# YuvalNirkin/hyperseg

Measured on AMD Instinct MI355X. Metric: frames/sec @ bs=1 HyperSeg-M 1024x512, higher is better.
Workload: dtype f32 storage and accumulation; level-4 inverted residual products as 3-term f16 splits (f32-class: 1.3e-7 of sum|a||b|; exact_f32 beside it)

## Files before the change

hyperseg_amd/_hip.py:

```python
import ctypes as C
import os

import torch

_LIB_PATH = os.environ.get('HS_HIP_LIB') or os.path.join(os.path.dirname(os.path.abspath(__file__)), 'lib',
                                                         'libhyperseg_hip.so')

ACT_NONE, ACT_RELU, ACT_RELU6, ACT_SWISH = 0, 1, 2, 3
PAD_MODES = {'zeros': 0, 'reflect': 1, 'replicate': 2, 'circular': 3}
PREV_NONE, PREV_SAME, PREV_BILINEAR = 0, 1, 2

_STATUS = {-1: 'bad argument', -2: 'feature map does not tile into the weight grid (H % fh or W % fw != 0)',
           -3: 'unsupported shape', -4: 'tile does not fit the LDS'}


class HipLibraryError(RuntimeError):
    pass


class StageInputC(C.Structure):
    _fields_ = [('skip', C.c_void_p), ('prev', C.c_void_p),
                ('batch', C.c_int32), ('H', C.c_int32), ('W', C.c_int32),
                ('c_skip', C.c_int32), ('c_prev', C.c_int32),
                ('Hp', C.c_int32), ('Wp', C.c_int32),
# ... 150 lines not shown
        'hs_frame_rotate_fwd': ([vp, i32, i32, i32, i32, vp, i32, i32, C.c_uint32, C.c_uint32, vp, vp, vp], C.c_int),
        'hs_label_rotate_fwd': ([vp, i32, i32, i32, i32, vp, i32, i32, i32, i32, vp, i32, vp], C.c_int),
        'hs_resize_tables_ragged_fwd': ([vp, i32, i32, i32, i32, i32, i32, i32, vp, vp, vp, vp, vp], C.c_int),
        'hs_color_jitter_ragged_fwd': ([vp, i32, i32, i32, i32, vp, vp, vp, vp, vp], C.c_int),
        'hs_frame_resize_ragged_fwd': ([vp, i32, i32, i32, i32, vp, vp, vp, vp, i32, i32, i32, vp, vp], C.c_int),
        'hs_label_resize_ragged_fwd': ([vp, i32, i32, i32, i32, vp, vp, vp, i32, i32, vp, vp], C.c_int),
        'hs_frame_rotate_ragged_fwd': ([vp, i32, i32, i32, i32, vp, vp, vp, i32, i32, C.c_uint32, C.c_uint32, vp, vp, vp], C.c_int),
        'hs_label_rotate_ragged_fwd': ([vp, i32, i32, i32, vp, vp, vp, i32, i32, i32, i32, vp, i32, vp], C.c_int),
        'hs_mbconv_expand_dw_fwd': ([vp, i32, i32, i32, i32, vp, i32, vp, vp, vp, i32, i32, i32, i32, i32, i32, vp, vp, vp, vp, vp], C.c_int),
        'hs_se_gate_fwd': ([vp, i32, i32, i32, C.c_float, vp, vp, i32, vp, vp, vp, vp, vp, i32, vp, vp, vp], C.c_int),
        'hs_gemm_split_kp': ([i32], C.c_int),
        'hs_gemm_split_fwd': ([vp, vp, vp, vp, vp, i32, vp, vp, i32, i32, i32, i32, i32, vp], C.c_int),
        'hs_gemm_split_conv2x2_fwd': ([vp, vp, vp, vp, i32, vp, vp, i32, i32, i32, i32, i32, i32, vp], C.c_int),
        'hs_gemm_split_up2_fwd': ([vp, vp, vp, vp, i32, vp, i32, i32, i32, i32, i32, i32, vp], C.c_int),
        'hs_pooled_shift_fwd': ([vp, i32, C.c_float, vp, vp, vp, i32, i32, vp], C.c_int),
    }
    for name, (argtypes, restype) in sig.items():
        fn = getattr(lib, name)
        fn.argtypes, fn.restype = argtypes, restype
    if lib.hs_version() != 1:
        raise HipLibraryError(f'ABI mismatch: library reports version {lib.hs_version()}, binding expects 1')
    return lib


lib = _load()
EXPORTS = ['hs_version', 'hs_build_info', 'hs_signal2weights_fwd', 'hs_signal2weights_multi_fwd', 'hs_s2w_pack_floats', 'hs_s2w_pack_fwd', 'hs_bank_pack_fwd', 'hs_bn_fold_fwd',
           'hs_patch_conv_fwd', 'hs_patch_conv_s2w_fwd', 'hs_k1_chain_workspace', 'hs_k1_chain_fwd', 'hs_decoder_chain_workspace', 'hs_decoder_chain_fwd', 'hs_meta_conv_fwd', 'hs_meta_conv_bwd', 'hs_patch_conv_gen_fwd', 'hs_patch_ir_fwd', 'hs_patch_ir_v0_fwd', 'hs_patch_ir_v0_ws_fwd', 'hs_patch_ir_v0_workspace', 'hs_patch_ir_route', 'hs_ir_tile_map', 'hs_upsample_bilinear_fwd', 'hs_upsample_argmax_fwd',
           'hs_stage_input_fwd', 'hs_depthwise_conv_fwd', 'hs_depthwise_pool_blocks', 'hs_stem_conv_fwd', 'hs_stem_dw_fwd', 'hs_mbconv_tiles', 'hs_mbconv_expand_dw_fwd', 'hs_se_gate_fwd', 'hs_depthwise_conv_se_fwd', 'hs_mbconv_expand_dw_se_fwd', 'hs_se_tail_workspace', 'hs_se_tail_tails', 'hs_mbconv_se_workgroups', 'hs_pointwise_conv_fwd', 'hs_affine_act_fwd', 'hs_gemm_split_kp', 'hs_gemm_split_fwd', 'hs_gemm_split_conv2x2_fwd', 'hs_gemm_split_up2_fwd', 'hs_pooled_shift_fwd', 'hs_patch_conv_bwd_input',
           'hs_patch_conv_bwd_weight', 'hs_halo_tiles_fwd', 'hs_halo_tiles_bwd', 'hs_tile_interior_fwd', 'hs_tile_interior_bwd', 'hs_dw_tiles_fwd', 'hs_dw_tiles_bwd_in', 'hs_dw_tiles_bwd_w',
           'hs_s2w_train_fwd', 'hs_s2w_train_workspace', 'hs_s2w_train_bwd', 'hs_cross_entropy_fwd', 'hs_cross_entropy_bwd', 'hs_cross_entropy_typed_fwd', 'hs_cross_entropy_typed_bwd', 'hs_bootstrapped_ce_fwd', 'hs_bootstrapped_ce_bwd', 'hs_bootstrap_mean_workspace', 'hs_bootstrap_mean_fwd', 'hs_bootstrap_mean_bwd', 'hs_bootstrap_mean_batched_fwd', 'hs_bootstrap_mean_batched_bwd', 'hs_bn_train_workspace', 'hs_bn_train_stats_fwd', 'hs_dw_tiles_bn_fwd', 'hs_dw_tiles_bn_bwd_w', 'hs_patch_conv_bn_fwd', 'hs_patch_conv_bn_bwd_w', 'hs_adam_blocks', 'hs_adam_step', 'hs_bootstrap_mean_of_batch_fwd', 'hs_bootstrap_mean_of_batch_bwd', 'hs_upsample_bilinear_bwd', 'hs_upsample_bilinear_typed_bwd', 'hs_upsample_bilinear_bf16_fwd', 'hs_stage_input_typed_fwd', 'hs_bank_unpack_fwd', 'hs_bn_act_train_fwd',
           'hs_bn_act_train_bwd', 'hs_dw_tiles_bn_bwd_in_partials', 'hs_dw_tiles_bn_bwd_in', 'hs_bn_act_train_bwd_apply', 'hs_patch_conv_plain_fwd', 'hs_patch_conv_plain_bwd_in', 'hs_patch_conv_plain_bwd_w',
           'hs_upsample_bilinear_f16_fwd', 'hs_adam_step_amp', 'hs_eval_max_classes', 'hs_upsample_confusion_fwd', 'hs_confusion_fwd', 'hs_upsample2_confusion_fwd',
           'hs_image_ingest_fwd', 'hs_stem_dw_u8_fwd', 'hs_overlay_fwd', 'hs_upsample_overlay_fwd',
           'hs_frame_resize_fwd', 'hs_label_resize_fwd', 'hs_resize_tables_fwd', 'hs_frame_resize_batch_fwd', 'hs_label_resize_batch_fwd', 'hs_color_jitter_fwd', 'hs_frame_rotate_fwd', 'hs_label_rotate_fwd',
           'hs_resize_tables_ragged_fwd', 'hs_color_jitter_ragged_fwd', 'hs_frame_resize_ragged_fwd', 'hs_label_resize_ragged_fwd', 'hs_frame_rotate_ragged_fwd', 'hs_label_rotate_ragged_fwd',
           'hs_cross_entropy_score_fwd', 'hs_upsample_ce_confusion_fwd']


def check(status, what):
    if status == 0:
        return
    if status < 0:
        raise HipLibraryError(f'{what}: {_STATUS.get(status, status)}')
    raise HipLibraryError(f'{what}: HIP launch failed with hipError_t {status}')


def dev_ptr(t, name='tensor', dtype=torch.float32):
    if t is None:
        return None
    if not isinstance(t, torch.Tensor):
        raise TypeError(f'{name} must be a torch.Tensor')
# ... 30 lines not shown
```

hyperseg_amd/csrc/hs_gemm_split.hip:

```cpp
#include "hs_common.h"
#include <type_traits>

namespace hs {

using half8 = __attribute__((ext_vector_type(8))) _Float16;
using gs_f32x4 = __attribute__((ext_vector_type(4))) float;

__device__ __forceinline__ int gs_exp_of(float m) { return min(max(__float_as_int(m) >> 23, 27), 254); }
__device__ __forceinline__ float gs_scale_of(int eb) { return __int_as_float((268 - eb) << 23); }
__device__ __forceinline__ float gs_inv_scale_of(int eb) { return __int_as_float((eb - 14) << 23); }

struct GemmSplitArgs {
    const _Float16* __restrict__ wf;
    const float* __restrict__ w_inv;
    const float* __restrict__ gate; const float* __restrict__ x;
    const float* shift;
    const float* residual;
    float* y;
    int M, K, KST, N, act;
    int conv_wo;
    float* pool_partial;
    int up2_wo;
};

#ifndef HS_GS_NARROW_MAX_WG
#define HS_GS_NARROW_MAX_WG 128
#endif

#ifndef HS_GS_TALL_MIN_WG
#define HS_GS_TALL_MIN_WG 257
#endif

template <int KS, int NWV, bool FAST, int NS, int MT, int NCH, bool PATCH>
__global__ __launch_bounds__(64 * NWV)
void gemm_split_kernel(GemmSplitArgs a) {
    extern __shared__ __attribute__((aligned(16))) float gs_red[];
    constexpr int nthr = 64 * NWV, nwv = NWV;
    constexpr int NP = 16 * NS, NR = 16 * MT, NE = NR * NP;
    const int tid = threadIdx.x, lane = tid & 63, wave = tid >> 6;
    const int lrow = lane & 15, kg = lane >> 4;
    const int n0 = blockIdx.x * NP, r0 = blockIdx.y * MT, b = blockIdx.z;
    const float* __restrict__ xb = a.x + (size_t)b * a.K * a.N;
    const float* __restrict__ gb = a.gate ? a.gate + (size_t)b * a.K : nullptr;
    float* yb = a.y + (size_t)b * a.M * a.N * (a.up2_wo > 0 ? 4 : 1);
    const float* rb = a.residual ? a.residual + (size_t)b * a.M * a.N : nullptr;
    const int rt_max = (a.M + 15) >> 4;

    using gs_f32x2 = __attribute__((ext_vector_type(2))) float;
    const int ncol0 = min(n0 + NS * lrow, a.N - (FAST && !PATCH && NS == 2 ? 2 : 1)), ncol1 = min(n0 + NS * lrow + 1, a.N - 1);
    float xv[NCH][NS][KS][8];
    if constexpr (PATCH) {
        const int oy = ncol0 / a.conv_wo, ox = ncol0 - oy * a.conv_wo;
        const float* __restrict__ win = xb + (size_t)(2 * oy) * (2 * a.conv_wo) + 2 * ox;
        const int cmax = (a.K >> 2) - 1;
#pragma unroll
        for (int c = 0; c < NCH; ++c)
#pragma unroll
            for (int s = 0; s < KS; ++s)
#pragma unroll
// ... 149 lines not shown
                }
            }
            if (q + 2 < NCH * MT) { load_a(q + 2); __builtin_amdgcn_sched_barrier(0); }
#pragma unroll
            for (int t = 0; t < NS; ++t) {
#pragma unroll
                for (int r = 0; r < 4; ++r) {
                    const float v = c == 0 ? acc[t][r] * invb[t] : fmaf(acc[t][r], invb[t], tot[mt][t][r]);
                    if (c == NCH - 1) gs_red[(wave * NR + 16 * mt + 4 * kg + r) * NP + NS * lrow + t] = v;
                    else tot[mt][t][r] = v;
                }
            }
        }
    }
    __syncthreads();
    auto tail = [&](auto act_kind) {
        constexpr int ACT = decltype(act_kind)::value;
#pragma unroll
        for (int i = 0; i < TE; ++i) {
            const int e = tid + i * nthr;
            if (e < NE) {
                const int row = 16 * r0 + e / NP, col = n0 + (e & (NP - 1));
                float t = 0.0f;
#pragma unroll
                for (int w = 0; w < nwv; ++w) t += gs_red[w * NE + e];
                const bool live = row < a.M && col < a.N;
                float v = fmaf(t, wi[i], sh[i]);
                if constexpr (ACT == HS_ACT_SWISH) v = swishf(v);
                else if constexpr (ACT == HS_ACT_RELU) v = fmaxf(v, 0.0f);
                else if constexpr (ACT == HS_ACT_RELU6) v = fminf(fmaxf(v, 0.0f), 6.0f);
                v += yo[i];
                if (live) {
                    if (a.up2_wo > 0) {
                        const int oy = col / a.up2_wo, ox = col - oy * a.up2_wo;
                        float* dst = yb + (size_t)row * (4 * a.N) + (size_t)(2 * oy) * (2 * a.up2_wo) + 2 * ox;
                        *reinterpret_cast<gs_f32x2*>(dst) = gs_f32x2{v, v};
                        *reinterpret_cast<gs_f32x2*>(dst + 2 * a.up2_wo) = gs_f32x2{v, v};
                    } else {
                        yb[(size_t)row * a.N + col] = v;
                    }
                }
                if constexpr (NP == 16) {
                    if (a.pool_partial) {
                        const float rs = rowsum16(live ? v : 0.0f);
                        if ((e & 15) == 0 && row < a.M) a.pool_partial[((size_t)b * a.M + row) * gridDim.x + blockIdx.x] = rs;
                    }
                }
            }
        }
    };
    if (a.act == HS_ACT_SWISH) tail(std::integral_constant<int, HS_ACT_SWISH>{});
    else if (a.act == HS_ACT_NONE) tail(std::integral_constant<int, HS_ACT_NONE>{});
    else if (a.act == HS_ACT_RELU) tail(std::integral_constant<int, HS_ACT_RELU>{});
    else tail(std::integral_constant<int, HS_ACT_RELU6>{});
}

__global__ __launch_bounds__(256)
void pooled_shift_kernel(const float* __restrict__ partial, int nblk, float inv_p, const float* __restrict__ wb,
                         const float* __restrict__ shift, float* __restrict__ out, int M, int C) {
    extern __shared__ float ps_mean[];
    const int tid = threadIdx.x, lane = tid & 63, wave = tid >> 6;
    for (int c = tid; c < C; c += 256) {
        float t = 0.0f;
        for (int j = 0; j < nblk; ++j) t += partial[(size_t)c * nblk + j];
        ps_mean[c] = t * inv_p;
    }
    __syncthreads();
    const int r0 = 16 * blockIdx.x + 4 * wave;
    float acc[4] = {0.f, 0.f, 0.f, 0.f};
// ... 20 lines not shown
    return ks <= 5;
}

}

using namespace hs;

extern "C" int hs_gemm_split_kp(int32_t c_in) {
    int nwv, ks, nch;
    if (c_in <= 0 || !gemm_split_plan(c_in, nwv, ks, nch)) return HS_ERR_UNSUPPORTED;
    return nwv * nch * ks * 32;
}

static int launch_gemm_split_plain(const void* w_frag, const float* w_inv, const float* gate, const float* x, const float* shift,
                                   int32_t act, const float* residual, float* y, int32_t batch, int32_t c_out, int32_t c_in,
                                   int32_t kp, int32_t pixels, int up2_wo, void* stream) {
    if (!w_frag || !w_inv || !x || !y || batch <= 0 || c_out <= 0 || c_in <= 0 || pixels <= 0) return HS_ERR_BAD_ARG;
    if (act < 0 || act > 3) return HS_ERR_BAD_ARG;
    int nwv, ks, nch;
    if (!gemm_split_plan(c_in, nwv, ks, nch)) return HS_ERR_UNSUPPORTED;
    if (kp != nwv * nch * ks * 32 || (ks > 1 && nwv != 8)) return HS_ERR_BAD_ARG;
    if (batch > 65535 || (c_out + 31) / 32 > 65535) return HS_ERR_UNSUPPORTED;
    GemmSplitArgs a{(const _Float16*)w_frag, w_inv, gate, x, shift, residual, y, c_out, c_in, kp / 32, pixels, act, 0, nullptr, up2_wo};
    dim3 grid((pixels + 31) / 32, ((c_out + 15) / 16 + 1) / 2, batch);
    const size_t wgs = (size_t)grid.x * grid.y * grid.z;
    const bool narrow = wgs <= HS_GS_NARROW_MAX_WG && pixels > 16;
    const bool tall = wgs >= HS_GS_TALL_MIN_WG && c_out > 32;
    if (narrow) grid.x = (pixels + 15) / 16;
    if (tall) grid.y = ((c_out + 15) / 16 + 3) / 4;
    const size_t lds = (size_t)nwv * (narrow ? 512 : tall ? 2048 : 1024) * sizeof(float);
    hipStream_t s = (hipStream_t)stream;
    const bool fast = (c_in & 7) == 0 && (pixels & 1) == 0 && c_in >= 8;
#define HS_GS_(KSV, NWV, F) do { \
        if (narrow) hipLaunchKernelGGL((gemm_split_kernel<KSV, NWV, F, 1, 2, 1, false>), grid, dim3(64 * NWV), lds, s, a); \
        else if (tall) hipLaunchKernelGGL((gemm_split_kernel<KSV, NWV, F, 2, 4, 1, false>), grid, dim3(64 * NWV), lds, s, a); \
        else hipLaunchKernelGGL((gemm_split_kernel<KSV, NWV, F, 2, 2, 1, false>), grid, dim3(64 * NWV), lds, s, a); } while (0)
#define HS_GS(KSV, NWV) do { if (fast) HS_GS_(KSV, NWV, true); else HS_GS_(KSV, NWV, false); } while (0)
    if (nch == 2) {
        if (!fast || up2_wo > 0) return HS_ERR_UNSUPPORTED;
        grid.x = (pixels + 15) / 16; grid.y = ((c_out + 15) / 16 + 1) / 2;
        const size_t lds2 = (size_t)8 * 512 * sizeof(float);
#define HS_GS2(KSV) hipLaunchKernelGGL((gemm_split_kernel<KSV, 8, true, 1, 2, 2, false>), grid, dim3(512), lds2, s, a)
        switch (ks) { case 3: HS_GS2(3); break; case 4: HS_GS2(4); break; case 5: HS_GS2(5); break; default: return HS_ERR_UNSUPPORTED; }
#undef HS_GS2
        return launch_status();
    }
    switch (ks) {
        case 1: if (nwv == 2) HS_GS(1, 2); else if (nwv == 4) HS_GS(1, 4); else HS_GS(1, 8); break;
        case 2: HS_GS(2, 8); break;
        case 3: HS_GS(3, 8); break;
        case 4: HS_GS(4, 8); break;
        default: HS_GS(5, 8); break;
// ... 2 lines not shown
#undef HS_GS_
    return launch_status();
}

extern "C" int hs_gemm_split_fwd(const void* w_frag, const float* w_inv, const float* gate, const float* x,
                                 const float* shift, int32_t act, const float* residual, float* y,
                                 int32_t batch, int32_t c_out, int32_t c_in, int32_t kp, int32_t pixels, void* stream) {
    return launch_gemm_split_plain(w_frag, w_inv, gate, x, shift, act, residual, y, batch, c_out, c_in, kp, pixels, 0, stream);
}

extern "C" int hs_gemm_split_up2_fwd(const void* w_frag, const float* w_inv, const float* x, const float* shift, int32_t act,
                                     float* y, int32_t batch, int32_t c_out, int32_t c_in, int32_t kp, int32_t Ho, int32_t Wo,
                                     void* stream) {
    if (Ho <= 0 || Wo <= 0 || (((size_t)y) & 7) != 0) return HS_ERR_BAD_ARG;
    return launch_gemm_split_plain(w_frag, w_inv, nullptr, x, shift, act, nullptr, y, batch, c_out, c_in, kp, Ho * Wo, Wo, stream);
}

extern "C" int hs_pooled_shift_fwd(const float* partial, int32_t nblk, float inv_pixels, const float* wb, const float* shift,
                                   float* shift_out, int32_t rows, int32_t channels, void* stream) {
    if (!partial || !wb || !shift || !shift_out || nblk <= 0 || rows <= 0 || channels <= 0) return HS_ERR_BAD_ARG;
    if (channels > 8192) return HS_ERR_UNSUPPORTED;
    hipLaunchKernelGGL(pooled_shift_kernel, dim3((rows + 15) / 16), dim3(256), (size_t)channels * sizeof(float), (hipStream_t)stream,
                       partial, nblk, inv_pixels, wb, shift, shift_out, rows, channels);
    return launch_status();
}

extern "C" int hs_gemm_split_conv2x2_fwd(const void* w_frag, const float* w_inv, const float* x, const float* shift, int32_t act,
                                         float* y, float* pool_partial, int32_t batch, int32_t c_out, int32_t c_in, int32_t kp,
                                         int32_t Ho, int32_t Wo, void* stream) {
    if (!w_frag || !w_inv || !x || !y || batch <= 0 || c_out <= 0 || c_in <= 0 || Ho <= 0 || Wo <= 0) return HS_ERR_BAD_ARG;
// ... 27 lines not shown
```

hyperseg_amd/functional.py:

```python
import collections
import ctypes as C
import functools
import os
import threading

import torch

from . import _hip
from ._hip import ACT_NONE, ACT_RELU, ACT_RELU6, PAD_MODES

BN_EPS_DEFAULT = 1e-5
DTYPE_CODES = {torch.float32: 0, torch.bfloat16: 1, torch.float16: 2}
S2W_TRAIN_MAX_LAYERS = 8
COSCHEDULE_BANKS = os.environ.get('HS_COSCHEDULE_BANKS', '0') == '1'


def _round_up(n, m):
    return (n + m - 1) // m * m


def _device_of(a):
    if isinstance(a, torch.Tensor):
        return a.device
    if isinstance(a, (StageInput, BankRef, SignalRef, U8Frame)):
# ... 1036 lines not shown
        raise ValueError(f'input has {cin} channels, the weight {sw.c_in}')
    shape = (b, sw.c_out, 2 * h, 2 * w)
    if out is None:
        out = torch.empty(shape, device=x.device, dtype=torch.float32)
    elif tuple(out.shape) != shape:
        raise ValueError(f'out has shape {tuple(out.shape)}, expected {shape}')
    if shift is not None and shift.numel() != sw.c_out:
        raise ValueError(f'shift has {shift.numel()} entries, expected {sw.c_out}')
    st = _hip.lib.hs_gemm_split_up2_fwd(_hip.dev_ptr(sw.frag, 'w_frag', torch.float16), _hip.dev_ptr(sw.inv, 'w_inv'),
                                        _hip.dev_ptr(x, 'x'), _hip.dev_ptr(shift, 'shift') if shift is not None else None,
                                        int(act), _hip.dev_ptr(out, 'out'), b, sw.c_out, cin, sw.kp, h, w, _hip.stream_ptr())
    _hip.check(st, 'hs_gemm_split_up2_fwd')
    return out


@_on_operand_device
def pooled_shift(pool_partial, pixels, wb, shift):
    _, c, nblk = pool_partial.shape
    m = shift.numel()
    if pool_partial.shape[0] != 1 or tuple(wb.shape) != (m, c):
        raise ValueError(f'pool_partial {tuple(pool_partial.shape)} / wb {tuple(wb.shape)} / shift {m}: expected (1, C, nblk), (M, C), M')
    out = torch.empty(m, device=shift.device, dtype=torch.float32)
    st = _hip.lib.hs_pooled_shift_fwd(_hip.dev_ptr(pool_partial, 'pool_partial'), nblk, 1.0 / pixels, _hip.dev_ptr(wb, 'wb'),
                                      _hip.dev_ptr(shift, 'shift'), _hip.dev_ptr(out, 'shift_out'), m, c, _hip.stream_ptr())
    _hip.check(st, 'hs_pooled_shift_fwd')
    return out


@_on_operand_device
def upsample_bilinear(x, size, out=None):
# ... 793 lines not shown
```

hyperseg_amd/models/backbones/efficientnet.py:

```python
import math
from functools import partial

import torch
import torch.nn as nn
import torch.nn.functional as F

_B0_STAGES = [
    (1, 3, 1, 32, 16, 1),
    (6, 3, 2, 16, 24, 2),
    (6, 5, 2, 24, 40, 2),
    (6, 3, 2, 40, 80, 3),
    (6, 5, 1, 80, 112, 3),
    (6, 5, 2, 112, 192, 4),
    (6, 3, 1, 192, 320, 1),
]
_SCALING = {
    'efficientnet-b0': (1.0, 1.0, 224, 0.2), 'efficientnet-b1': (1.0, 1.1, 240, 0.2),
    'efficientnet-b2': (1.1, 1.2, 260, 0.3), 'efficientnet-b3': (1.2, 1.4, 300, 0.3),
    'efficientnet-b4': (1.4, 1.8, 380, 0.4), 'efficientnet-b5': (1.6, 2.2, 456, 0.4),
    'efficientnet-b6': (1.8, 2.6, 528, 0.5), 'efficientnet-b7': (2.0, 3.1, 600, 0.5),
}
_BN_MOMENTUM, _BN_EPS, _SE_RATIO, _DIVISOR = 0.01, 1e-3, 0.25, 8


# ... 47 lines not shown
        mid = in_f * expand
        bn = partial(nn.BatchNorm2d, momentum=_BN_MOMENTUM, eps=_BN_EPS)
        if expand != 1:
            self._expand_conv = SamePadConv2d(in_f, mid, 1, image_size=image_size, bias=False)
            self._bn0 = bn(mid)
        self._depthwise_conv = SamePadConv2d(mid, mid, kernel, stride, image_size=image_size, groups=mid, bias=False)
        self._bn1 = bn(mid)
        squeezed = max(1, int(in_f * _SE_RATIO))
        self._se_reduce = SamePadConv2d(mid, squeezed, 1, image_size=1)
        self._se_expand = SamePadConv2d(squeezed, mid, 1, image_size=1)
        self._project_conv = SamePadConv2d(mid, out_f, 1, image_size=_out_size(image_size, stride), bias=False)
        self._bn2 = bn(out_f)
        self._fused_dw = None
        self._fused_active = None

    def forward(self, inputs, drop_connect_rate=None):
        active = self._fused_active if self._fused_active is not None else _inference_only(self, inputs)
        if self._fused_dw is not None and active:
            return self._fused_dw(inputs, self)
        x = inputs
        if self.expand != 1:
            x = F.silu(self._bn0(self._expand_conv(x)))
        x = F.silu(self._bn1(self._depthwise_conv(x)))
        gate = self._se_expand(F.silu(self._se_reduce(F.adaptive_avg_pool2d(x, 1))))
        x = self._bn2(self._project_conv(torch.sigmoid(gate) * x))
        if self.stride == 1 and self.in_f == self.out_f:
            if drop_connect_rate and self.training:
                keep = 1.0 - drop_connect_rate
                mask = torch.floor(keep + torch.rand(x.shape[0], 1, 1, 1, dtype=x.dtype, device=x.device))
                x = x / keep * mask
            x = x + inputs
        return x


# ... 77 lines not shown
            return self._extract_features_list(inputs, use)
        finally:
            for blk in self._blocks:
                blk._fused_active = None

    def _extract_features_list(self, inputs, use):
        f0 = self._blocks[0]._fused_dw if len(self._blocks) else None
        if self._fused_stem is not None and use and f0 is not None and getattr(f0, '_stem', None) is not None:
            x = inputs
        elif self._fused_stem is not None and use:
            x = self._fused_stem(inputs)
        else:
            x = F.silu(self._bn0(self._conv_stem(inputs)))
        feats = []
        n = len(self._blocks)
        for idx, block in enumerate(self._blocks):
            rate = self.drop_connect_rate * float(idx) / n if self.drop_connect_rate else None
            x = block(x, drop_connect_rate=rate)
            if self._res_feat_mask[idx]:
                fc = getattr(self, f'_feat_fc_{len(feats)}', None) if self.out_feat_scale is not None else None
                fused = self._fused_fc is not None and use and str(len(feats)) in self._fused_fc
                feats.append(self._fused_fc[str(len(feats))](x) if fused else (x if fc is None else fc(x)))
        if self._fused_head is not None and use:
            x = self._fused_head(x)
        else:
            x = F.silu(self._bn1(self._conv_head(x)))
        if self.pool:
            x = self._avg_pooling(x).flatten(1)
        x = self._dropout(x)
        if self._fc is not None:
            x = self._fc(x)
        feats.append(x)
        return feats

    def forward(self, inputs):
        feats = self.extract_features_list(inputs)
        return feats if self.return_features else feats[-1]

# ... 7 lines not shown
```

hyperseg_amd/utils/inference.py:

```python
import contextlib
import os

import torch
import torch.nn as nn

from ..models._common import Blend, Epilogue, HyperGenBase, Score


class InputNorm:

    LAYOUTS = ('hwc', 'chw')

    def __init__(self, mean=(0.485, 0.456, 0.406), std=(0.229, 0.224, 0.225), layout='hwc'):
        if layout not in self.LAYOUTS:
            raise ValueError(f'layout {layout!r}: expected one of {self.LAYOUTS}')
        self.mean = torch.as_tensor(mean, dtype=torch.float32).flatten().clone()
        self.std = torch.as_tensor(std, dtype=torch.float32).flatten().clone()
        if self.mean.numel() != 3 or self.std.numel() != 3:
            raise ValueError('mean and std must hold one value per channel of a 3-channel frame')
        if bool((self.std == 0).any()):
            raise ValueError('std must be non-zero')
        self.layout = layout
        values = torch.arange(256, dtype=torch.float32)
        self._tables = {torch.device('cpu'): ((values.div(255)[None, :] - self.mean[:, None]) / self.std[:, None]).contiguous()}
# ... 179 lines not shown
            _fold(mods[i], mods[i + 1])
            seq[i + 1] = nn.Identity()
            n += 1
    return n


def _bn_affine(bn):
    with torch.no_grad():
        scale = bn.weight / torch.sqrt(bn.running_var + bn.eps)
        shift = bn.bias - bn.running_mean * scale
    return scale.detach().clone(), shift.detach().clone()


SPLIT_GEMM_MAX_K = int(os.environ.get('HS_SPLIT_GEMM_MAX_K', '1280'))
STEM_DW = os.environ.get('HS_STEM_DW', '1') != '0'
FUSE_EXPAND_MIN_PIXELS = int(os.environ.get('HS_FUSE_EXPAND_MIN_PIXELS', '2048'))
FUSE_EXPAND_MAX_CIN = int(os.environ.get('HS_FUSE_EXPAND_MAX_CIN', '40'))


LEAN_MFMA_MAX_CIN = int(os.environ.get('HS_LEAN_MFMA_MAX_CIN', '16'))
PW_MFMA_MAX_CIN = int(os.environ.get('HS_PW_MFMA_MAX_CIN', '96'))
PW_MFMA_MIN_PIXELS = int(os.environ.get('HS_PW_MFMA_MIN_PIXELS', '8192'))
GEMM_LT_MIN_PIXELS = int(os.environ.get('HS_GEMM_LT_MIN_PIXELS', '16384'))


@contextlib.contextmanager
def gemm_library(pixels, batch=1):
    want = os.environ.get('HS_BLAS') or ('cublaslt' if (pixels >= GEMM_LT_MIN_PIXELS or batch > 1) else 'cublas')
    prev = torch.backends.cuda.preferred_blas_library()
    torch.backends.cuda.preferred_blas_library(want)
# ... 3 lines not shown
        torch.backends.cuda.preferred_blas_library(prev)


class FusedPointwise(nn.Module):

    def __init__(self, conv, bn, act=0):
        super().__init__()
        assert conv.kernel_size == (1, 1) and conv.stride == (1, 1) and conv.groups == 1 and conv.bias is None
        scale, shift = _bn_affine(bn)
        self.register_buffer('scale', scale, persistent=False)
        self.register_buffer('shift', shift, persistent=False)
        self._conv = [conv]
        self.act = act
        self.split_gemm = False
        self._split = {}

    @property
    def conv(self):
        return self._conv[0]

    def split_weights(self, with_scale, device):
        from .. import functional as HF
        srcs = (self.conv.weight, self.scale) if with_scale else (self.conv.weight,)
        key, ver = (bool(with_scale), device), HF._key(*srcs)
        hit = self._split.get(key)
        if hit is None or hit[0] != ver:
            hit = (ver, HF.gemm_split_weights(self.conv.weight, self.scale if with_scale else None, max_k=SPLIT_GEMM_MAX_K), HF.producer_stream(self.conv.weight.device))
            HF.publish_ready(self.conv.weight.device)
            self._split[key] = hit
        elif hit[1] is not None:
# ... 11 lines not shown
    @staticmethod
    def mfma_covers(channels, pixels):
        return channels <= PW_MFMA_MAX_CIN and pixels >= PW_MFMA_MIN_PIXELS

    def raw(self, x):
        b, cin, h, w = x.shape
        if self.split_gemm:
            sw = self.split_weights(False, x.device)
            if sw is not None:
                from .. import functional as HF
                return HF.gemm_split(sw, x.contiguous())
        with gemm_library(h * w, b):
            if b == 1:
                return torch.mm(self.conv.weight.view(-1, cin), x.view(cin, h * w)).view(1, -1, h, w)
            return torch.bmm(self.conv.weight.view(1, -1, cin).expand(b, -1, -1), x.view(b, cin, h * w)).view(b, -1, h, w)

    def forward(self, x, gate=None, residual=None):
        import torch.nn.functional as F
        from .. import functional as HF
        conv = self.conv
        x = x.contiguous()
        b, cin, h, w = x.shape
        if self.uses_mfma(x):
            return HF.pointwise_conv(x, conv.weight, gate, self.scale, self.shift, self.act, residual)
        if (h * w) % 4 != 0:
            raise NotImplementedError('feature maps with H*W % 4 != 0')
        sw = self.split_weights(True, x.device) if self.split_gemm else None
        if sw is not None:
            return HF.gemm_split(sw, x, gate=gate, shift=self.shift, act=self.act, residual=residual)
        if gate is None:
# ... 58 lines not shown
            self.expand.absorb_input_offset(in_offset)
        with torch.no_grad():
            carried = self.project.shift.clone()
            if self.skip and in_offset is not None:
                carried += in_offset.to(carried.device)
            self.defer_shift = bool(defer_shift)
            self.out_offset = carried.clone() if defer_shift else None
            self.project.shift.copy_(torch.zeros_like(carried) if defer_shift else carried)

    def takes_image(self):
        return self._stem is not None and STEM_DW

    def fuses_expand(self, x, ho, wo):
        return self.expand is not None and x.shape[1] <= FUSE_EXPAND_MAX_CIN and ho * wo >= FUSE_EXPAND_MIN_PIXELS

    def forward(self, inputs, blk):
        from .. import functional as HF
        pre = None
        if self._stem is not None and inputs.shape[1] == 3:
            stem = self._stem[0]
            img = inputs.contiguous()
            pre = HF.stem_dw(img, stem.w28, stem.scale, stem.shift, stem.pad_t, stem.pad_l, stem.out_size(img),
                             blk._depthwise_conv.weight, self.pad_t, self.pad_l, self.scale, self.shift, pool=True) if STEM_DW else None
            if pre is None and isinstance(img, HF.U8Frame):
                img = img.float_image()
            inputs = pre[0] if pre is not None else stem(img)
        x = inputs.contiguous()
        b, _, h, w = x.shape
        ho = (h + self.pad_h - self.k) // self.stride + 1
        wo = (w + self.pad_w - self.k) // self.stride + 1
        lean = True
# ... 6 lines not shown
        cmid = blk._depthwise_conv.weight.shape[0]
        lean_gemm = lean and (cmid > LEAN_MFMA_MAX_CIN if self.defer_shift else not proj.mfma_covers(cmid, ho * wo))
        folds = lean_gemm and not (proj.split_gemm and proj.split_weights(True, x.device) is not None)
        se = (self._red_w, red.bias, self._exp_t, exp.bias) if self.se_tail and not folds else None
        if pre is not None:
            out = (pre[0], pre[1], False) if se is not None else pre
        elif self.fuses_expand(x, ho, wo):
            out = HF.mbconv_expand_dw(x, self.expand.conv.weight, self.expand.scale, self.expand.shift,
                                      blk._depthwise_conv.weight, self.stride, self.pad_t, self.pad_l, (ho, wo),
                                      self.scale, self.shift, pool=True, se=se)
        else:
            in_scale = in_shift = None
            if self.expand is not None:
                if lean and not self.expand.uses_mfma(x):
                    in_scale, in_shift = self.expand.scale, self.expand.shift
                    x = self.expand.raw(x)
                else:
                    x = self.expand(x)
            out = HF.depthwise_conv_bn_act(x, blk._depthwise_conv.weight, self.stride, self.pad_t, self.pad_l,
                                           (ho, wo), self.scale, self.shift, act=3, pool=True,
                                           in_scale=in_scale, in_shift=in_shift, se=se)
        y, pooled, gated = out if se is not None else (out[0], out[1], False)

        def se_gate(**fold):
            if gated and not fold:
                return pooled
            return HF.se_gate(pooled, b, ho * wo, red.weight, red.bias, self._exp_t, exp.bias, **fold)
        skip = inputs.contiguous() if self.skip else None
        if lean_gemm:
            sw = proj.split_weights(True, y.device) if proj.split_gemm else None
            if sw is not None:
# ... 120 lines not shown
                if sw_up is not None:
                    y = HF.gemm_split(sw_up, skip.contiguous(), shift=shift, act=HF.ACT_RELU)
                else:
                    y = HF.affine_act_(torch.mm(wgt[:, :half], skip.view(half, sh * sw)).view(1, half, sh, sw), scale, shift, HF.ACT_RELU)
                pooled_const = False
            else:
                y = torch.mm(wgt, torch.cat((skip, t), dim=1).view(cin, sh * sw)).view(1, half, sh, sw)
                y = HF.affine_act_(y, scale, shift, HF.ACT_RELU)
            if level > 0:
                t = wm.upsample(y)
            else:
                signal[:, half:].view(half, sh, 2, sw, 2).copy_(y.view(half, sh, 1, sw, 1).expand(half, sh, 2, sw, 2))
        return signal


def _fuse_backbone(bb):
    blocks = list(bb._blocks)
    offset, tap = None, 0
    bb._fused_fc = nn.ModuleDict()
    for idx, blk in enumerate(blocks):
        conv = blk._depthwise_conv
        ok = conv.kernel_size[0] in (3, 5) and conv.stride[0] in (1, 2) and isinstance(blk._bn1, nn.BatchNorm2d)
        tapped = bb._res_feat_mask[idx]
        fc = getattr(bb, f'_feat_fc_{tap}', None) if (tapped and bb.out_feat_scale is not None) else None
        if ok:
            nxt = blocks[idx + 1] if idx + 1 < len(blocks) else None
            nxt_ok = nxt is None or (nxt.expand != 1 and nxt._depthwise_conv.kernel_size[0] in (3, 5)
                                     and isinstance(nxt._bn1, nn.BatchNorm2d))
            defer = nxt_ok and (not tapped or isinstance(fc, nn.Sequential))
            blk._fused_dw = FusedMBConv(blk, in_offset=offset, defer_shift=defer)
# ... 316 lines not shown
```

include/hyperseg_hip.h:

```cpp
#ifndef HYPERSEG_HIP_H
#define HYPERSEG_HIP_H

#include <stdint.h>

#ifdef __cplusplus
extern "C" {
#endif

#define HS_ABI_VERSION 1

typedef enum {
    HS_OK = 0,
    HS_ERR_BAD_ARG = -1,
    HS_ERR_NOT_DIVISIBLE = -2,
    HS_ERR_UNSUPPORTED = -3,
    HS_ERR_LDS = -4
} hs_status;

typedef enum { HS_ACT_NONE = 0, HS_ACT_RELU = 1, HS_ACT_RELU6 = 2, HS_ACT_SWISH = 3 } hs_act;
typedef enum { HS_PAD_ZEROS = 0, HS_PAD_REFLECT = 1, HS_PAD_REPLICATE = 2, HS_PAD_CIRCULAR = 3 } hs_pad_mode;
typedef enum { HS_PREV_NONE = 0, HS_PREV_SAME = 1, HS_PREV_BILINEAR = 2 } hs_prev_mode;

typedef struct {
    const float* skip;
// ... 270 lines not shown
                          const float* gate, const float* scale, const float* shift, int32_t act, const float* residual,
                          float* y, void* stream);

int hs_affine_act_fwd(const float* x, int32_t batch, int32_t channels, int32_t pixels, const float* scale,
                      const float* shift, int32_t act, const float* residual, float* y, void* stream);

int hs_gemm_split_kp(int32_t c_in);
int hs_gemm_split_fwd(const void* w_frag, const float* w_inv, const float* gate, const float* x, const float* shift,
                      int32_t act, const float* residual, float* y, int32_t batch, int32_t c_out, int32_t c_in, int32_t kp,
                      int32_t pixels, void* stream);
int hs_gemm_split_conv2x2_fwd(const void* w_frag, const float* w_inv, const float* x, const float* shift, int32_t act, float* y,
                              float* pool_partial, int32_t batch, int32_t c_out, int32_t c_in, int32_t kp, int32_t Ho,
                              int32_t Wo, void* stream);
int hs_gemm_split_up2_fwd(const void* w_frag, const float* w_inv, const float* x, const float* shift, int32_t act, float* y,
                          int32_t batch, int32_t c_out, int32_t c_in, int32_t kp, int32_t Ho, int32_t Wo, void* stream);
int hs_pooled_shift_fwd(const float* partial, int32_t nblk, float inv_pixels, const float* wb, const float* shift,
                        float* shift_out, int32_t rows, int32_t channels, void* stream);

int hs_halo_tiles_fwd(int32_t dtype, const void* x, int32_t batch, int32_t channels, int32_t H, int32_t W, int32_t fh, int32_t fw,
                      void* tiled, int32_t patch_major, void* stream);
int hs_halo_tiles_bwd(int32_t dtype, const void* dtiled, int32_t batch, int32_t channels, int32_t H, int32_t W, int32_t fh, int32_t fw,
                      void* dx, int32_t patch_major, void* stream);
int hs_tile_interior_fwd(int32_t dtype, const void* tiled, int32_t batch, int32_t channels, int32_t H, int32_t W, int32_t fh,
                         int32_t fw, void* y, void* stream);
int hs_tile_interior_bwd(int32_t dtype, const void* dy, int32_t batch, int32_t channels, int32_t H, int32_t W, int32_t fh, int32_t fw,
                         void* dtiled, void* stream);
int hs_dw_tiles_fwd(int32_t dtype, const void* tiled, const float* bank, int64_t ld, int32_t batch, int32_t channels, int32_t H, int32_t W,
                    int32_t fh, int32_t fw, void* y, int32_t patch_major, void* stream);
int hs_dw_tiles_bwd_in(int32_t dtype, const void* dy, const float* bank, int64_t ld, int32_t batch, int32_t channels, int32_t H, int32_t W,
                       int32_t fh, int32_t fw, void* dtiled, int32_t patch_major, void* stream);
// ... 97 lines not shown
```

Baseline: 1350.

## Fuse feature-tap reducer with next block's expand conv in one split GEMM

At backbone feature taps, the 1x1 reducer conv and the following block's raw expand conv (or the head conv) read the same input. They are now run as a single split-f16 GEMM over concatenated weights, with a per-row activation and an optional second output buffer. The expanded result is handed to the next block so it skips its own expand GEMM. This saves one kernel launch and a second read of the activation at each tap, at the cost of a more complex tail with dual activation passes, cached concatenated weights, and new control flow through the backbone forward.

```diff
diff --git a/hyperseg_amd/_hip.py b/hyperseg_amd/_hip.py
--- a/hyperseg_amd/_hip.py
+++ b/hyperseg_amd/_hip.py
@@ -188,6 +188,7 @@
         'hs_gemm_split_conv2x2_fwd': ([vp, vp, vp, vp, i32, vp, vp, i32, i32, i32, i32, i32, i32, vp], C.c_int),
         'hs_gemm_split_up2_fwd': ([vp, vp, vp, vp, i32, vp, i32, i32, i32, i32, i32, i32, vp], C.c_int),
         'hs_pooled_shift_fwd': ([vp, i32, C.c_float, vp, vp, vp, i32, i32, vp], C.c_int),
+        'hs_gemm_split_pair_fwd': ([vp, vp, vp, vp, i32, i32, vp, vp, i32, i32, i32, i32, i32, i32, vp], C.c_int),
     }
     for name, (argtypes, restype) in sig.items():
         fn = getattr(lib, name)
@@ -208,7 +209,7 @@
            'hs_image_ingest_fwd', 'hs_stem_dw_u8_fwd', 'hs_overlay_fwd', 'hs_upsample_overlay_fwd',
            'hs_frame_resize_fwd', 'hs_label_resize_fwd', 'hs_resize_tables_fwd', 'hs_frame_resize_batch_fwd', 'hs_label_resize_batch_fwd', 'hs_color_jitter_fwd', 'hs_frame_rotate_fwd', 'hs_label_rotate_fwd',
            'hs_resize_tables_ragged_fwd', 'hs_color_jitter_ragged_fwd', 'hs_frame_resize_ragged_fwd', 'hs_label_resize_ragged_fwd', 'hs_frame_rotate_ragged_fwd', 'hs_label_rotate_ragged_fwd',
-           'hs_cross_entropy_score_fwd', 'hs_upsample_ce_confusion_fwd']
+           'hs_cross_entropy_score_fwd', 'hs_upsample_ce_confusion_fwd', 'hs_gemm_split_pair_fwd']
 
 
 def check(status, what):
diff --git a/hyperseg_amd/csrc/hs_gemm_split.hip b/hyperseg_amd/csrc/hs_gemm_split.hip
--- a/hyperseg_amd/csrc/hs_gemm_split.hip
+++ b/hyperseg_amd/csrc/hs_gemm_split.hip
@@ -21,7 +21,11 @@
     int conv_wo;
     float* pool_partial;
     int up2_wo;
+    int m_split = 0, act2 = 0;
+    float* y2 = nullptr;
 };
+
+enum { GS_PLAIN = 0, GS_PAIR = 1 };
 
 #ifndef HS_GS_NARROW_MAX_WG
 #define HS_GS_NARROW_MAX_WG 128
@@ -31,7 +35,7 @@
 #define HS_GS_TALL_MIN_WG 257
 #endif
 
-template <int KS, int NWV, bool FAST, int NS, int MT, int NCH, bool PATCH>
+template <int KS, int NWV, bool FAST, int NS, int MT, int NCH, bool PATCH, int EXTRA = GS_PLAIN>
 __global__ __launch_bounds__(64 * NWV)
 void gemm_split_kernel(GemmSplitArgs a) {
     extern __shared__ __attribute__((aligned(16))) float gs_red[];
@@ -42,7 +46,7 @@
     const int n0 = blockIdx.x * NP, r0 = blockIdx.y * MT, b = blockIdx.z;
     const float* __restrict__ xb = a.x + (size_t)b * a.K * a.N;
     const float* __restrict__ gb = a.gate ? a.gate + (size_t)b * a.K : nullptr;
-    float* yb = a.y + (size_t)b * a.M * a.N * (a.up2_wo > 0 ? 4 : 1);
+    float* yb = a.y + (size_t)b * (EXTRA == GS_PAIR && a.y2 ? a.m_split : a.M) * a.N * (a.up2_wo > 0 ? 4 : 1);
     const float* rb = a.residual ? a.residual + (size_t)b * a.M * a.N : nullptr;
     const int rt_max = (a.M + 15) >> 4;
 
@@ -222,13 +226,14 @@
         }
     }
     __syncthreads();
-    auto tail = [&](auto act_kind) {
+    auto tail = [&](auto act_kind, int part) {
         constexpr int ACT = decltype(act_kind)::value;
 #pragma unroll
         for (int i = 0; i < TE; ++i) {
             const int e = tid + i * nthr;
             if (e < NE) {
                 const int row = 16 * r0 + e / NP, col = n0 + (e & (NP - 1));
+                if constexpr (EXTRA == GS_PAIR) { if (part != 0 && (row >= a.m_split) != (part == 2)) continue; }
                 float t = 0.0f;
 #pragma unroll
                 for (int w = 0; w < nwv; ++w) t += gs_red[w * NE + e];
@@ -244,11 +249,13 @@
                         float* dst = yb + (size_t)row * (4 * a.N) + (size_t)(2 * oy) * (2 * a.up2_wo) + 2 * ox;
                         *reinterpret_cast<gs_f32x2*>(dst) = gs_f32x2{v, v};
                         *reinterpret_cast<gs_f32x2*>(dst + 2 * a.up2_wo) = gs_f32x2{v, v};
+                    } else if (EXTRA == GS_PAIR && a.y2 && row >= a.m_split) {
+                        a.y2[((size_t)b * (a.M - a.m_split) + (row - a.m_split)) * a.N + col] = v;
                     } else {
                         yb[(size_t)row * a.N + col] = v;
                     }
                 }
-                if constexpr (NP == 16) {
+                if constexpr (NP == 16 && EXTRA != GS_PAIR) {
                     if (a.pool_partial) {
                         const float rs = rowsum16(live ? v : 0.0f);
                         if ((e & 15) == 0 && row < a.M) a.pool_partial[((size_t)b * a.M + row) * gridDim.x + blockIdx.x] = rs;
@@ -257,10 +264,23 @@
             }
         }
     };
-    if (a.act == HS_ACT_SWISH) tail(std::integral_constant<int, HS_ACT_SWISH>{});
-    else if (a.act == HS_ACT_NONE) tail(std::integral_constant<int, HS_ACT_NONE>{});
-    else if (a.act == HS_ACT_RELU) tail(std::integral_constant<int, HS_ACT_RELU>{});
-    else tail(std::integral_constant<int, HS_ACT_RELU6>{});
+    if constexpr (EXTRA == GS_PAIR) {
+        const int lo = 16 * r0;
+        const bool straddles = lo < a.m_split && lo + NR > a.m_split;
+        for (int pass = 0; pass < (straddles ? 2 : 1); ++pass) {
+            const int part = straddles ? pass + 1 : 0;
+            const int act = (straddles ? pass == 1 : lo >= a.m_split) ? a.act2 : a.act;
+            if (act == HS_ACT_SWISH) tail(std::integral_constant<int, HS_ACT_SWISH>{}, part);
+            else if (act == HS_ACT_NONE) tail(std::integral_constant<int, HS_ACT_NONE>{}, part);
+            else if (act == HS_ACT_RELU) tail(std::integral_constant<int, HS_ACT_RELU>{}, part);
+            else tail(std::integral_constant<int, HS_ACT_RELU6>{}, part);
+        }
+    } else {
+        if (a.act == HS_ACT_SWISH) tail(std::integral_constant<int, HS_ACT_SWISH>{}, 0);
+        else if (a.act == HS_ACT_NONE) tail(std::integral_constant<int, HS_ACT_NONE>{}, 0);
+        else if (a.act == HS_ACT_RELU) tail(std::integral_constant<int, HS_ACT_RELU>{}, 0);
+        else tail(std::integral_constant<int, HS_ACT_RELU6>{}, 0);
+    }
 }
 
 __global__ __launch_bounds__(256)
@@ -311,9 +331,10 @@
 
 static int launch_gemm_split_plain(const void* w_frag, const float* w_inv, const float* gate, const float* x, const float* shift,
                                    int32_t act, const float* residual, float* y, int32_t batch, int32_t c_out, int32_t c_in,
-                                   int32_t kp, int32_t pixels, int up2_wo, void* stream) {
+                                   int32_t kp, int32_t pixels, int up2_wo, void* stream, int extra = GS_PLAIN,
+                                   const GemmSplitArgs* ext = nullptr) {
     if (!w_frag || !w_inv || !x || !y || batch <= 0 || c_out <= 0 || c_in <= 0 || pixels <= 0) return HS_ERR_BAD_ARG;
-    if (act < 0 || act > 3) return HS_ERR_BAD_ARG;
+    if (act < 0 || act > 3 || (extra != GS_PLAIN && !ext)) return HS_ERR_BAD_ARG;
     int nwv, ks, nch;
     if (!gemm_split_plan(c_in, nwv, ks, nch)) return HS_ERR_UNSUPPORTED;
     if (kp != nwv * nch * ks * 32 || (ks > 1 && nwv != 8)) return HS_ERR_BAD_ARG;
@@ -327,12 +348,23 @@
     if (tall) grid.y = ((c_out + 15) / 16 + 3) / 4;
     const size_t lds = (size_t)nwv * (narrow ? 512 : tall ? 2048 : 1024) * sizeof(float);
     hipStream_t s = (hipStream_t)stream;
+    if (extra == GS_PAIR) { a.m_split = ext->m_split; a.act2 = ext->act2; a.y2 = ext->y2; }
     const bool fast = (c_in & 7) == 0 && (pixels & 1) == 0 && c_in >= 8;
 #define HS_GS_(KSV, NWV, F) do { \
         if (narrow) hipLaunchKernelGGL((gemm_split_kernel<KSV, NWV, F, 1, 2, 1, false>), grid, dim3(64 * NWV), lds, s, a); \
         else if (tall) hipLaunchKernelGGL((gemm_split_kernel<KSV, NWV, F, 2, 4, 1, false>), grid, dim3(64 * NWV), lds, s, a); \
         else hipLaunchKernelGGL((gemm_split_kernel<KSV, NWV, F, 2, 2, 1, false>), grid, dim3(64 * NWV), lds, s, a); } while (0)
 #define HS_GS(KSV, NWV) do { if (fast) HS_GS_(KSV, NWV, true); else HS_GS_(KSV, NWV, false); } while (0)
+    if (extra == GS_PAIR) {
+        if (!fast || nch != 1 || ks > 2) return HS_ERR_UNSUPPORTED;
+#define HS_GX(KSV, NWV) do { \
+        if (narrow) hipLaunchKernelGGL((gemm_split_kernel<KSV, NWV, true, 1, 2, 1, false, GS_PAIR>), grid, dim3(64 * NWV), lds, s, a); \
+        else if (tall) hipLaunchKernelGGL((gemm_split_kernel<KSV, NWV, true, 2, 4, 1, false, GS_PAIR>), grid, dim3(64 * NWV), lds, s, a); \
+        else hipLaunchKernelGGL((gemm_split_kernel<KSV, NWV, true, 2, 2, 1, false, GS_PAIR>), grid, dim3(64 * NWV), lds, s, a); } while (0)
+        if (ks == 2) HS_GX(2, 8); else if (nwv == 2) HS_GX(1, 2); else if (nwv == 4) HS_GX(1, 4); else HS_GX(1, 8);
+#undef HS_GX
+        return launch_status();
+    }
     if (nch == 2) {
         if (!fast || up2_wo > 0) return HS_ERR_UNSUPPORTED;
         grid.x = (pixels + 15) / 16; grid.y = ((c_out + 15) / 16 + 1) / 2;
@@ -365,6 +397,16 @@
                                      void* stream) {
     if (Ho <= 0 || Wo <= 0 || (((size_t)y) & 7) != 0) return HS_ERR_BAD_ARG;
     return launch_gemm_split_plain(w_frag, w_inv, nullptr, x, shift, act, nullptr, y, batch, c_out, c_in, kp, Ho * Wo, Wo, stream);
+}
+
+extern "C" int hs_gemm_split_pair_fwd(const void* w_frag, const float* w_inv, const float* x, const float* shift, int32_t act,
+                                      int32_t act2, float* y, float* y2, int32_t batch, int32_t c_out, int32_t m_split,
+                                      int32_t c_in, int32_t kp, int32_t pixels, void* stream) {
+    if (m_split <= 0 || m_split >= c_out || act2 < 0 || act2 > 3) return HS_ERR_BAD_ARG;
+    if (m_split & 15) return HS_ERR_UNSUPPORTED;
+    GemmSplitArgs ext{};
+    ext.m_split = m_split; ext.act2 = act2; ext.y2 = y2;
+    return launch_gemm_split_plain(w_frag, w_inv, nullptr, x, shift, act, nullptr, y, batch, c_out, c_in, kp, pixels, 0, stream, GS_PAIR, &ext);
 }
 
 extern "C" int hs_pooled_shift_fwd(const float* partial, int32_t nblk, float inv_pixels, const float* wb, const float* shift,
diff --git a/hyperseg_amd/functional.py b/hyperseg_amd/functional.py
--- a/hyperseg_amd/functional.py
+++ b/hyperseg_amd/functional.py
@@ -1074,6 +1074,45 @@
     return out
 
 
+class SplitPair:
+    __slots__ = ('frag', 'inv', 'm_a', 'm_b', 'c_in', 'kp')
+
+    def __init__(self, frag, inv, m_a, m_b, c_in, kp):
+        self.frag, self.inv, self.m_a, self.m_b, self.c_in, self.kp = frag, inv, m_a, m_b, c_in, kp
+
+
+@torch.no_grad()
+def gemm_split_pair_weights(sw_a, sw_b):
+    if sw_a is None or sw_b is None or sw_a.c_out % 16 != 0 or sw_a.c_in != sw_b.c_in or sw_a.kp != sw_b.kp:
+        return None
+    return SplitPair(torch.cat((sw_a.frag, sw_b.frag), 0).contiguous(), torch.cat((sw_a.inv, sw_b.inv)).contiguous(),
+                     sw_a.c_out, sw_b.c_out, sw_a.c_in, sw_a.kp)
+
+
+@_on_operand_device
+def gemm_split_pair(pair, x, shift=None, act_a=ACT_NONE, act_b=ACT_NONE):
+    b, cin, h, w = x.shape
+    if cin != pair.c_in:
+        raise ValueError(f'input has {cin} channels, the weights {pair.c_in}')
+    m = pair.m_a + pair.m_b
+    if shift is not None and shift.numel() != m:
+        raise ValueError(f'shift has {shift.numel()} entries, expected {m}')
+    if b == 1:
+        both = torch.empty((1, m, h, w), device=x.device, dtype=torch.float32)
+        ya, yb, y2 = both[:, :pair.m_a], both[:, pair.m_a:], None
+    else:
+        ya = torch.empty((b, pair.m_a, h, w), device=x.device, dtype=torch.float32)
+        yb = y2 = torch.empty((b, pair.m_b, h, w), device=x.device, dtype=torch.float32)
+    st = _hip.lib.hs_gemm_split_pair_fwd(_hip.dev_ptr(pair.frag, 'w_frag', torch.float16), _hip.dev_ptr(pair.inv, 'w_inv'), _hip.dev_ptr(x, 'x'),
+                                         _hip.dev_ptr(shift, 'shift') if shift is not None else None, int(act_a), int(act_b),
+                                         _hip.dev_ptr(ya, 'out'), _hip.dev_ptr(y2, 'out2') if y2 is not None else None,
+                                         b, m, pair.m_a, cin, pair.kp, h * w, _hip.stream_ptr())
+    if st == -3:
+        return None
+    _hip.check(st, 'hs_gemm_split_pair_fwd')
+    return ya, yb
+
+
 @_on_operand_device
 def pooled_shift(pool_partial, pixels, wb, shift):
     _, c, nblk = pool_partial.shape
diff --git a/hyperseg_amd/models/backbones/efficientnet.py b/hyperseg_amd/models/backbones/efficientnet.py
--- a/hyperseg_amd/models/backbones/efficientnet.py
+++ b/hyperseg_amd/models/backbones/efficientnet.py
@@ -85,10 +85,10 @@
         self._fused_dw = None
         self._fused_active = None
 
-    def forward(self, inputs, drop_connect_rate=None):
+    def forward(self, inputs, drop_connect_rate=None, expanded=None):
         active = self._fused_active if self._fused_active is not None else _inference_only(self, inputs)
         if self._fused_dw is not None and active:
-            return self._fused_dw(inputs, self)
+            return self._fused_dw(inputs, self, expanded)
         x = inputs
         if self.expand != 1:
             x = F.silu(self._bn0(self._expand_conv(x)))
@@ -196,14 +196,23 @@
             x = F.silu(self._bn0(self._conv_stem(inputs)))
         feats = []
         n = len(self._blocks)
+        expanded = head = None
         for idx, block in enumerate(self._blocks):
             rate = self.drop_connect_rate * float(idx) / n if self.drop_connect_rate else None
-            x = block(x, drop_connect_rate=rate)
+            x = block(x, drop_connect_rate=rate) if expanded is None else block(x, drop_connect_rate=rate, expanded=expanded)
+            expanded = None
             if self._res_feat_mask[idx]:
                 fc = getattr(self, f'_feat_fc_{len(feats)}', None) if self.out_feat_scale is not None else None
                 fused = self._fused_fc is not None and use and str(len(feats)) in self._fused_fc
-                feats.append(self._fused_fc[str(len(feats))](x) if fused else (x if fc is None else fc(x)))
-        if self._fused_head is not None and use:
+                if fused:
+                    from ...utils.inference import tap_with_next
+                    feat, expanded, head = tap_with_next(self, idx, self._fused_fc[str(len(feats))], x)
+                    feats.append(feat)
+                else:
+                    feats.append(x if fc is None else fc(x))
+        if head is not None:
+            x = head
+        elif self._fused_head is not None and use:
             x = self._fused_head(x)
         else:
             x = F.silu(self._bn1(self._conv_head(x)))
diff --git a/hyperseg_amd/utils/inference.py b/hyperseg_amd/utils/inference.py
--- a/hyperseg_amd/utils/inference.py
+++ b/hyperseg_amd/utils/inference.py
@@ -217,6 +217,7 @@
 
 SPLIT_GEMM_MAX_K = int(os.environ.get('HS_SPLIT_GEMM_MAX_K', '1280'))
 STEM_DW = os.environ.get('HS_STEM_DW', '1') != '0'
+PAIR_REDUCER = os.environ.get('HS_PAIR_REDUCER', '1') != '0'
 FUSE_EXPAND_MIN_PIXELS = int(os.environ.get('HS_FUSE_EXPAND_MIN_PIXELS', '2048'))
 FUSE_EXPAND_MAX_CIN = int(os.environ.get('HS_FUSE_EXPAND_MAX_CIN', '40'))
 
@@ -250,6 +251,7 @@
         self.act = act
         self.split_gemm = False
         self._split = {}
+        self._pair = {}
 
     @property
     def conv(self):
@@ -291,6 +293,38 @@
             if b == 1:
                 return torch.mm(self.conv.weight.view(-1, cin), x.view(cin, h * w)).view(1, -1, h, w)
             return torch.bmm(self.conv.weight.view(1, -1, cin).expand(b, -1, -1), x.view(b, cin, h * w)).view(b, -1, h, w)
+
+    def forward_pair(self, x, other, other_raw):
+        from .. import functional as HF
+        b, cin, h, w = x.shape
+        if not (PAIR_REDUCER and self.split_gemm and other.split_gemm) or (h * w) % 4 != 0 or not x.is_contiguous():
+            return None
+        if self.uses_mfma(x) or (not other_raw and other.uses_mfma(x)):
+            return None
+        sw_s, sw_o = self.split_weights(True, x.device), other.split_weights(not other_raw, x.device)
+        if sw_s is None or sw_o is None:
+            return None
+        other_first = sw_o.c_out % 16 == 0
+        key = (id(sw_s), id(sw_o), HF._key(self.shift, other.shift))
+        hit = self._pair.get(x.device)
+        if hit is None or hit[0] != key:
+            pair = HF.gemm_split_pair_weights(*((sw_o, sw_s) if other_first else (sw_s, sw_o)))
+            shift = None
+            if pair is not None:
+                sh_o = torch.zeros_like(other.shift) if other_raw else other.shift
+                shift = torch.cat((sh_o, self.shift) if other_first else (self.shift, sh_o)).to(x.device).contiguous()
+            hit = (key, pair, shift, HF.producer_stream(x.device), (sw_s, sw_o))
+            HF.publish_ready(x.device)
+            self._pair[x.device] = hit
+        elif hit[1] is not None:
+            HF.adopt((hit[1].frag, hit[1].inv, hit[2]), x.device, hit[3])
+        if hit[1] is None:
+            return None
+        act_o = 0 if other_raw else other.act
+        got = HF.gemm_split_pair(hit[1], x, shift=hit[2], act_a=act_o if other_first else self.act, act_b=self.act if other_first else act_o)
+        if got is None:
+            return None
+        return (got[1], got[0]) if other_first else got
 
     def forward(self, x, gate=None, residual=None):
         import torch.nn.functional as F
@@ -379,7 +413,14 @@
     def fuses_expand(self, x, ho, wo):
         return self.expand is not None and x.shape[1] <= FUSE_EXPAND_MAX_CIN and ho * wo >= FUSE_EXPAND_MIN_PIXELS
 
-    def forward(self, inputs, blk):
+    def takes_raw_expand(self, x):
+        if self.expand is None or self._stem is not None:
+            return False
+        ho = (x.shape[2] + self.pad_h - self.k) // self.stride + 1
+        wo = (x.shape[3] + self.pad_w - self.k) // self.stride + 1
+        return not self.fuses_expand(x, ho, wo) and not self.expand.uses_mfma(x)
+
+    def forward(self, inputs, blk, expanded=None):
         from .. import functional as HF
         pre = None
         if self._stem is not None and inputs.shape[1] == 3:
@@ -416,7 +457,7 @@
             if self.expand is not None:
                 if lean and not self.expand.uses_mfma(x):
                     in_scale, in_shift = self.expand.scale, self.expand.shift
-                    x = self.expand.raw(x)
+                    x = expanded if expanded is not None else self.expand.raw(x)
                 else:
                     x = self.expand(x)
             out = HF.depthwise_conv_bn_act(x, blk._depthwise_conv.weight, self.stride, self.pad_t, self.pad_l,
@@ -567,6 +608,22 @@
         return signal
 
 
+def tap_with_next(bb, idx, reducer, x):
+    blocks = bb._blocks
+    got = None
+    if idx + 1 < len(blocks):
+        nxt = blocks[idx + 1]._fused_dw
+        if nxt is not None and nxt.takes_raw_expand(x):
+            got = reducer.forward_pair(x.contiguous(), nxt.expand, True)
+            if got is not None:
+                return got[0], got[1], None
+    elif bb._fused_head is not None:
+        got = reducer.forward_pair(x.contiguous(), bb._fused_head, False)
+        if got is not None:
+            return got[0], None, got[1]
+    return reducer(x), None, None
+
+
 def _fuse_backbone(bb):
     blocks = list(bb._blocks)
     offset, tap = None, 0
diff --git a/include/hyperseg_hip.h b/include/hyperseg_hip.h
--- a/include/hyperseg_hip.h
+++ b/include/hyperseg_hip.h
@@ -308,6 +308,9 @@
                               int32_t Wo, void* stream);
 int hs_gemm_split_up2_fwd(const void* w_frag, const float* w_inv, const float* x, const float* shift, int32_t act, float* y,
                           int32_t batch, int32_t c_out, int32_t c_in, int32_t kp, int32_t Ho, int32_t Wo, void* stream);
+int hs_gemm_split_pair_fwd(const void* w_frag, const float* w_inv, const float* x, const float* shift, int32_t act, int32_t act2,
+                           float* y, float* y2, int32_t batch, int32_t c_out, int32_t m_split, int32_t c_in, int32_t kp,
+                           int32_t pixels, void* stream);
 int hs_pooled_shift_fwd(const float* partial, int32_t nblk, float inv_pixels, const float* wb, const float* shift,
                         float* shift_out, int32_t rows, int32_t channels, void* stream);
 
```

Result: no change. 1356, median of 6 (+0.4%).
